# jpreprocess/jbonsai

Measured on AMD Instinct MI355X. Metric: 48 kHz PCM samples/sec (whole node), batched utterances, higher is better.
Workload: dtype f64

## Files before the change

jbonsai_amd/csrc/jb_mlpg.hip:

```cpp
#include "jb_device.h"

#include <cstdlib>
#include <type_traits>

namespace jb {

__device__ __forceinline__ uint32_t ps_scan_incl(uint32_t v, int lane)
{
#pragma unroll
    for (int o = 1; o < 64; o <<= 1) {
        const uint32_t u = (uint32_t)__shfl_up((int)v, o);
        if (lane >= o)
            v += u;
    }
    return v;
}

__global__ __launch_bounds__(64) void k_prep_states(BatchDev bd, StreamDev sd, int si)
{
    if ((int)blockIdx.x >= bd.B)
        return;
    const int b = (int)bd.order[blockIdx.x];
    const int lane = threadIdx.x;
    const UttDev *up = bd.utt + b;
// ... 1064 lines not shown
        if (p >= 0 && p < nch && lane < L) {
            const long l0 = lo(p);
            const double *ib = inb + (p % kFlIn) * NIN * kFlCT * LP;
            double *ob = outb + (p % kFlOut) * NOUT * kFlCT * LP;
            constexpr int kHalf = kFlCT / 2;
            const bool interior = l0 >= 2 && l0 + kFlCT + 2 <= (long)n;
#pragma unroll
            for (int h = 0; h < 2; h++) {
                double ivs[kHalf][NIN];
#pragma unroll
                for (int uu = 0; uu < kHalf; uu++) {
                    const int u = h * kHalf + uu;
                    const int tt = BACKWARD ? kFlCT - 1 - u : u;
#pragma unroll
                    for (int a = 0; a < NIN; a++)
                        ivs[uu][a] = ib[(a * kFlCT + tt) * LP + lane];
                }
                __builtin_amdgcn_sched_barrier(0);
                if (interior) {
#pragma unroll
                    for (int uu = 0; uu < kHalf; uu++) {
                        const int u = h * kHalf + uu;
                        const int tt = BACKWARD ? kFlCT - 1 - u : u;
                        double ov[NOUT];
                        step(std::true_type{}, (uint32_t)(l0 + tt), ivs[uu], ov);
#pragma unroll
                        for (int a = 0; a < NOUT; a++)
                            ob[(a * kFlCT + tt) * LP + lane] = ov[a];
                    }
                } else {
#pragma unroll
                    for (int uu = 0; uu < kHalf; uu++) {
                        const int u = h * kHalf + uu;
                        const int tt = BACKWARD ? kFlCT - 1 - u : u;
                        const long t = l0 + tt;
                        if (t >= 0 && t < (long)n) {
                            double ov[NOUT];
                            step(std::false_type{}, (uint32_t)t, ivs[uu], ov);
#pragma unroll
                            for (int a = 0; a < NOUT; a++)
                                ob[(a * kFlCT + tt) * LP + lane] = ov[a];
                        }
                    }
                }
                __builtin_amdgcn_sched_barrier(0);
            }
        }
    };
    auto phase_end = [&]() {
        asm volatile("s_waitcnt lgkmcnt(0)" ::: "memory");
        __builtin_amdgcn_s_barrier();
        asm volatile("" ::: "memory");
    };
    static_assert(kFlGroups == 3 && kFlOut == 3, "roles: park c-2 / drain c+2 fall on different groups for 3");
    for (int p = -2 - kFlGroups; p <= nch + 1; p++) {
        if (solver)
            solver_phase(p);
        else
            mover_phase(p);
        phase_end();
    }
}

template <int LMAX>
__global__ __launch_bounds__(kFlNT, 1) void k_mlpg_fb_lds(BatchDev bd, StreamDev sd, int si)
{
    extern __shared__ double lds[];
    const int b = (int)bd.order[blockIdx.x];
    const UttDev *up = bd.utt + b;
    const uint32_t n = sd.Tv[b];
    if (n == 0)
        return;
    const int L = sd.L;
    const uint64_t row0 = mt_row0(up, L);
    const uint64_t rs = up->mt_rs;
    if (threadIdx.x < 64)
        __builtin_amdgcn_s_setprio(3);
    else
        __builtin_amdgcn_s_setprio(2);
    {
        const double *const in[4] = {sd.A[0] + row0, sd.A[1] + row0, sd.A[2] + row0, sd.bvec + row0};
        double *const out[3] = {sd.F[1] + row0, sd.F[2] + row0, sd.g + row0};
        double p1_0 = 0, p1_1 = 0, p1_2 = 0, p2_0 = 0, p2_2 = 0, g1 = 0, g2 = 0;
        fl_pass<LMAX, 4, 3, false>(lds, in, out, n, L, rs,
                                   [&](auto interior, uint32_t t, const double (&iv)[4], double (&ov)[3]) {
            constexpr bool IN = decltype(interior)::value;
            double r0 = iv[0], r1 = iv[1], r2 = iv[2], g = iv[3];
            if (IN || t >= 1)
                r0 -= p1_1 * p1_1 * p1_0;
            if (IN || t >= 2)
                r0 -= p2_2 * p2_2 * p2_0;
            if (IN || t >= 1)
                r1 -= p1_1 * p1_2 * p1_0;
            const double rr = fb_rcp(r0);
            r1 = fb_div(r1, r0, rr);
            r2 = fb_div(r2, r0, rr);
            if (IN || t >= 1)
                g -= p1_1 * g1;
            if (IN || t >= 2)
                g -= p2_2 * g2;
            ov[0] = r1;
            ov[1] = r2;
            ov[2] = fb_div(g, r0, rr);
            p2_0 = p1_0;
            p2_2 = p1_2;
            g2 = g1;
            p1_0 = r0;
            p1_1 = r1;
            p1_2 = r2;
            g1 = g;
        });
    }
    __threadfence();
    __syncthreads();
    {
        const double *const in[3] = {sd.F[1] + row0, sd.F[2] + row0, sd.g + row0};
        double *const out[1] = {sd.par + row0};
        double q1 = 0, q2 = 0;
        fl_pass<LMAX, 3, 1, true>(lds, in, out, n, L, rs,
                                  [&](auto interior, uint32_t t, const double (&iv)[3], double (&ov)[1]) {
            constexpr bool IN = decltype(interior)::value;
            double p = iv[2];
            if (IN || t + 1 < n)
                p -= iv[0] * q1;
            if (IN || t + 2 < n)
                p -= iv[1] * q2;
            ov[0] = p;
            q2 = q1;
            q1 = p;
        });
    }
}

constexpr int kFrCh = 8;
constexpr int kFrPitch = kFrCh + 1;
__global__ __launch_bounds__(64) void k_mlpg_fb_runs(BatchDev bd, StreamDev sd, int si)
{
    const int b = (int)bd.order[blockIdx.y];
    const UttDev *up = bd.utt + b;
    const int lane = threadIdx.x;
    const uint32_t r = blockIdx.x * 64u + (uint32_t)lane;
    const uint32_t nr = sd.nruns[b];
    if (blockIdx.x * 64u >= nr)
        return;
    const uint64_t base = up->frame_off, sb = up->state_off;
    const uint32_t T = up->T;
    uint32_t k0 = 0, len = 0;
    if (r < nr) {
        const uint32_t t0 = sd.run_list[sb + r];
        const bool ok = t0 < T && sd.voiced[base + t0] && !(t0 > 0 && sd.voiced[base + t0 - 1]) &&
                        !(r > 0 && sd.run_list[sb + r - 1] == t0);
        if (ok) {
            const uint32_t s0 = sd.fstate[base + t0];
            k0 = sd.s_vpre[sb + s0] + (t0 - sd.s_start[sb + s0]);
            len = sd.s_rend[sb + s0] - t0 + 1;
        }
    }
    __shared__ uint32_t rk0[64], rlen[64];
    __shared__ double img[4][64][kFrPitch];
    rk0[lane] = k0;
    rlen[lane] = len;
    uint32_t maxlen = len;
    for (int o = 32; o > 0; o >>= 1)
        maxlen = max(maxlen, (uint32_t)__shfl_xor((int)maxlen, o));
    if (maxlen == 0)
        return;
    const uint32_t nch = (maxlen + kFrCh - 1) / kFrCh;
    auto wsync = [] {
        __builtin_amdgcn_fence(__ATOMIC_RELEASE, "wavefront");
        __builtin_amdgcn_wave_barrier();
        __builtin_amdgcn_fence(__ATOMIC_ACQUIRE, "wavefront");
    };
    wsync();
    const int sub = lane & 7, grp = lane >> 3;
    const double *const in4[4] = {sd.A[0] + base, sd.A[1] + base, sd.A[2] + base, sd.bvec + base};
    double *const f4[4] = {sd.F[0] + base, sd.F[1] + base, sd.F[2] + base, sd.g + base};
    auto fetch = [&](const double *const (&arr)[4], uint32_t c, double (&v)[4][8]) {
#pragma unroll
        for (int j = 0; j < 8; j++) {
            const int rr = 8 * j + grp;
            const uint32_t t = c * kFrCh + (uint32_t)sub;
            const bool in = t < rlen[rr];
            const uint64_t o = (uint64_t)rk0[rr] + (in ? t : 0u);
#pragma unroll
            for (int a = 0; a < 4; a++)
                v[a][j] = arr[a][o];
        }
    };
    auto park = [&](const double (&v)[4][8]) {
#pragma unroll
        for (int j = 0; j < 8; j++)
#pragma unroll
            for (int a = 0; a < 4; a++)
                img[a][8 * j + grp][sub] = v[a][j];
    };
    auto drain = [&](double *const *arr, int na, uint32_t c) {
#pragma unroll
        for (int j = 0; j < 8; j++) {
            const int rr = 8 * j + grp;
            const uint32_t t = c * kFrCh + (uint32_t)sub;
            if (t < rlen[rr]) {
                const uint64_t o = (uint64_t)rk0[rr] + t;
                for (int a = 0; a < na; a++)
                    arr[a][o] = img[a][rr][sub];
            }
        }
    };
    {
        double p1_0 = 0, p1_1 = 0, p1_2 = 0, p2_0 = 0, p2_2 = 0, g1 = 0, g2 = 0;
        double v[4][8];
        fetch(in4, 0, v);
        for (uint32_t c = 0; c < nch; c++) {
            wsync();
            park(v);
            if (c + 1 < nch)
                fetch(in4, c + 1, v);
            wsync();
            const uint32_t tb = c * kFrCh;
#pragma unroll
            for (int i = 0; i < kFrCh; i++) {
                const uint32_t t = tb + (uint32_t)i;
                if (t < len) {
                    double r0 = img[0][lane][i], r1 = img[1][lane][i], r2 = img[2][lane][i], g = img[3][lane][i];
                    if (t >= 1)
                        r0 -= p1_1 * p1_1 * p1_0;
                    if (t >= 2)
                        r0 -= p2_2 * p2_2 * p2_0;
                    if (t >= 1)
                        r1 -= p1_1 * p1_2 * p1_0;
                    const double rr = fb_rcp(r0);
                    r1 = fb_div(r1, r0, rr);
                    r2 = fb_div(r2, r0, rr);
                    if (t >= 1)
                        g -= p1_1 * g1;
                    if (t >= 2)
                        g -= p2_2 * g2;
                    img[0][lane][i] = r0;
                    img[1][lane][i] = r1;
                    img[2][lane][i] = r2;
                    img[3][lane][i] = g;
                    p2_0 = p1_0;
                    p2_2 = p1_2;
                    g2 = g1;
                    p1_0 = r0;
                    p1_1 = r1;
                    p1_2 = r2;
                    g1 = g;
                }
            }
            wsync();
            drain(f4, 4, c);
        }
    }
    __threadfence_block();
    wsync();
    {
        double q1 = 0, q2 = 0;
        double v[4][8];
        double *const p1[1] = {sd.par + base};
        const double *const fr4[4] = {sd.F[0] + base, sd.F[1] + base, sd.F[2] + base, sd.g + base};
        fetch(fr4, nch - 1, v);
        for (uint32_t c = nch; c-- > 0;) {
            wsync();
            park(v);
            if (c > 0)
                fetch(fr4, c - 1, v);
            wsync();
            const uint32_t tb = c * kFrCh;
#pragma unroll
            for (int i = kFrCh - 1; i >= 0; i--) {
                const uint32_t t = tb + (uint32_t)i;
                if (t < len) {
                    const double d = img[0][lane][i];
                    double p = fb_div(img[3][lane][i], d, fb_rcp(d));
                    if (t + 1 < len)
                        p -= img[1][lane][i] * q1;
                    if (t + 2 < len)
                        p -= img[2][lane][i] * q2;
                    img[0][lane][i] = p;
                    q2 = q1;
                    q1 = p;
                }
            }
            wsync();
            drain(p1, 1, c);
        }
    }
}

__device__ __forceinline__ double rl64(double v, int lane)
{
    int lo = __builtin_amdgcn_readlane(__double2loint(v), lane);
    int hi = __builtin_amdgcn_readlane(__double2hiint(v), lane);
    return __hiloint2double(hi, lo);
}
__device__ __forceinline__ double serial_add64(double acc, double v)
{
#pragma unroll
    for (int u = 0; u < 64; u++)
        acc += rl64(v, u);
    return acc;
}

#ifndef JB_VT_NB
#define JB_VT_NB 8
#endif
constexpr int kVtNB = JB_VT_NB;

__device__ __forceinline__ double serial_add_lds(double acc, const double *buf)
{
    const double2 *b2 = reinterpret_cast<const double2 *>(buf);
    double2 x[2][8];
#pragma unroll
    for (int u = 0; u < 8; u++)
        x[0][u] = b2[u];
#pragma unroll
    for (int g = 0; g < 4; g++) {
        if (g < 3) {
#pragma unroll
            for (int u = 0; u < 8; u++)
                x[(g + 1) & 1][u] = b2[8 * (g + 1) + u];
        }
        __builtin_amdgcn_sched_barrier(0);
#pragma unroll
        for (int u = 0; u < 8; u++) {
            acc += x[g & 1][u].x;
            acc += x[g & 1][u].y;
        }
        __builtin_amdgcn_sched_barrier(0);
    }
    return acc;
}

__device__ __forceinline__ void serial_add2_lds(double &acc_a, const double *buf_a, double &acc_b, const double *buf_b)
{
    const double2 *a2 = reinterpret_cast<const double2 *>(buf_a), *b2 = reinterpret_cast<const double2 *>(buf_b);
    double2 x[2][4], y[2][4];
#pragma unroll
    for (int u = 0; u < 4; u++) {
        x[0][u] = a2[u];
        y[0][u] = b2[u];
    }
#pragma unroll
    for (int g = 0; g < 8; g++) {
        if (g < 7) {
#pragma unroll
            for (int u = 0; u < 4; u++) {
                x[(g + 1) & 1][u] = a2[4 * (g + 1) + u];
                y[(g + 1) & 1][u] = b2[4 * (g + 1) + u];
            }
        }
        __builtin_amdgcn_sched_barrier(0);
#pragma unroll
        for (int u = 0; u < 4; u++) {
            acc_a += x[g & 1][u].x;
            acc_b += y[g & 1][u].x;
            acc_a += x[g & 1][u].y;
            acc_b += y[g & 1][u].y;
        }
        __builtin_amdgcn_sched_barrier(0);
    }
}

template <bool NONMSD>
__global__ __launch_bounds__(64) void k_mlpg_gv_vt(BatchDev bd, StreamDev sd, int si)
{
    const int m = blockIdx.x, b = (int)bd.order[blockIdx.y], lane = threadIdx.x;
    const UttDev *up = bd.utt + b;
    const StreamStatesDev st = up->st[si];
    const uint32_t n = sd.Tv[b];
    const uint32_t gvl = sd.gvlen[b];
    if (n == 0 || !(sd.use_gv && st.gv_mean && gvl > 0))
        return;
    const int L = sd.L;
    const uint64_t base = up->frame_off;
    const uint64_t o0 = base * (uint64_t)L + (uint64_t)m, Ls = (uint64_t)L;
#define IX(k) (o0 + (uint64_t)(k) * Ls)
    __shared__ __attribute__((aligned(16))) double sbuf[2][kVtNB][64];
    const uint8_t *sw = sd.vsw + base;
    const double *A0 = sd.A[0], *A1 = sd.A[1], *A2 = sd.A[2], *Bv = sd.bvec;
    double *Gv = sd.g, *Pv = sd.par, *Ov = sd.out;
    const double gv_mean = st.gv_mean[m] * st.gv_weight;
    const double gv_vari = st.gv_var[m];
    const double glen = (double)gvl;
    constexpr uint32_t STEP = 64u * kVtNB;

    double ssum = 0.0;
    for (uint32_t tb = 0; tb < n; tb += STEP) {
        double v[kVtNB];
#pragma unroll
        for (int q = 0; q < kVtNB; q++) {
            const uint32_t t = tb + 64u * q + (uint32_t)lane;
            v[q] = (t < n && sw[t]) ? Pv[IX(t)] : 0.0;
        }
        __syncthreads();
#pragma unroll
        for (int q = 0; q < kVtNB; q++)
            sbuf[0][q][lane] = v[q];
        __syncthreads();
#pragma unroll
        for (int q = 0; q < kVtNB; q++)
            if (tb + 64u * q < n)
                ssum = serial_add_lds(ssum, sbuf[0][q]);
    }
    double mean = ssum / glen;
    double vsum = 0.0;
    for (uint32_t tb = 0; tb < n; tb += STEP) {
        double v[kVtNB];
#pragma unroll
        for (int q = 0; q < kVtNB; q++) {
            const uint32_t t = tb + 64u * q + (uint32_t)lane;
            const bool on = t < n && sw[t];
            const double p = on ? Pv[IX(t)] : mean;
            v[q] = on ? (p - mean) * (p - mean) : 0.0;
        }
        __syncthreads();
#pragma unroll
        for (int q = 0; q < kVtNB; q++)
            sbuf[0][q][lane] = v[q];
        __syncthreads();
#pragma unroll
        for (int q = 0; q < kVtNB; q++)
            if (tb + 64u * q < n)
                vsum = serial_add_lds(vsum, sbuf[0][q]);
    }
    double vari = vsum / glen;
    {
        const double ratio = sqrt(gv_mean / vari);
        ssum = 0.0;
        for (uint32_t tb = 0; tb < n; tb += STEP) {
            double v[kVtNB];
#pragma unroll
            for (int q = 0; q < kVtNB; q++) {
                const uint32_t t = tb + 64u * q + (uint32_t)lane;
                const bool on = t < n && sw[t];
                double pn = 0.0;
                if (on) {
                    pn = ratio * (Pv[IX(t)] - mean) + mean;
                    Pv[IX(t)] = pn;
                }
                v[q] = pn;
            }
        __syncthreads();
#pragma unroll
        for (int q = 0; q < kVtNB; q++)
            sbuf[0][q][lane] = v[q];
        __syncthreads();
#pragma unroll
        for (int q = 0; q < kVtNB; q++)
            if (tb + 64u * q < n)
                ssum = serial_add_lds(ssum, sbuf[0][q]);
        }
    }
    double step = 0.1, prev = 0.0;
    const double length = (double)n;
    const double wgt = 1.0 / (double)((uint64_t)sd.W * (uint64_t)n);
    const double ll = (double)((uint64_t)n * (uint64_t)n);
    const double lm1 = (double)(n - 1);
    for (int it = 1; it <= 5; it++) {
        mean = ssum / glen;
        double hmmobj = 0.0;
        vsum = 0.0;
        __syncthreads();
        for (uint32_t tb = 0; tb < n; tb += STEP) {
            double vs[kVtNB], hv[kVtNB];
            double l_p0[kVtNB], l_pp1[kVtNB], l_pm1[kVtNB], l_pp2[kVtNB], l_pm2[kVtNB], l_a0[kVtNB],
                l_a1[kVtNB], l_a1m[kVtNB], l_a2[kVtNB], l_a2m[kVtNB], l_b[kVtNB];
            uint8_t l_sw[kVtNB];
#pragma unroll
            for (int q = 0; q < kVtNB; q++) {
                const uint32_t t = tb + 64u * q + (uint32_t)lane;
                const uint32_t tc = t < n ? t : n - 1;
                const uint32_t t1 = tc + 1 < n ? tc + 1 : n - 1, t2 = tc + 2 < n ? tc + 2 : n - 1;
                const uint32_t m1 = tc >= 1 ? tc - 1 : 0, m2 = tc >= 2 ? tc - 2 : 0;
                l_p0[q] = Pv[IX(tc)];
                l_pp1[q] = Pv[IX(t1)];
                l_pm1[q] = Pv[IX(m1)];
                l_pp2[q] = Pv[IX(t2)];
                l_pm2[q] = Pv[IX(m2)];
                l_a0[q] = A0[IX(tc)];
                l_a1[q] = A1[IX(tc)];
                l_a1m[q] = A1[IX(m1)];
                l_a2[q] = A2[IX(tc)];
                l_a2m[q] = A2[IX(m2)];
                l_b[q] = Bv[IX(tc)];
                l_sw[q] = sw[tc];
            }
#pragma unroll
            for (int q = 0; q < kVtNB; q++) {
                const uint32_t t = tb + 64u * q + (uint32_t)lane;
                vs[q] = hv[q] = 0.0;
                if (t < n) {
                    const double p0 = l_p0[q];
                    if (l_sw[q])
                        vs[q] = (p0 - mean) * (p0 - mean);
                    double g = l_a0[q] * p0;
                    if (t + 1 < n)
                        g += l_a1[q] * l_pp1[q];
                    if (t >= 1)
                        g += l_a1m[q] * l_pm1[q];
                    if (t + 2 < n)
                        g += l_a2[q] * l_pp2[q];
                    if (t >= 2)
                        g += l_a2m[q] * l_pm2[q];
                    Gv[IX(t)] = g;
                    hv[q] = 1.0 * wgt * p0 * (l_b[q] - 0.5 * g);
                }
            }
            __syncthreads();
#pragma unroll
            for (int q = 0; q < kVtNB; q++) {
                sbuf[0][q][lane] = vs[q];
                sbuf[1][q][lane] = hv[q];
            }
            __syncthreads();
#pragma unroll
            for (int q = 0; q < kVtNB; q++)
                if (tb + 64u * q < n) {
                    serial_add2_lds(vsum, sbuf[0][q], hmmobj, sbuf[1][q]);
                }
        }
        vari = vsum / glen;
        const double gvobj = -0.5 * 1.0 * vari * gv_vari * (vari - 2.0 * gv_mean);
        const double obj = -(hmmobj + gvobj);
        if (it > 1) {
            if (obj > prev)
                step *= 0.5;
            else if (obj < prev)
                step *= 1.2;
        }
        const double dv = -2.0 * gv_vari * (vari - gv_mean) / length;
        ssum = 0.0;
        __syncthreads();
        for (uint32_t tb = 0; tb < n; tb += STEP) {
            double sn[kVtNB];
            double l_p[kVtNB], l_a0[kVtNB], l_g[kVtNB], l_b[kVtNB];
            uint8_t l_sw[kVtNB];
#pragma unroll
            for (int q = 0; q < kVtNB; q++) {
                const uint32_t t = tb + 64u * q + (uint32_t)lane;
                const uint32_t tc = t < n ? t : n - 1;
                l_p[q] = Pv[IX(tc)];
                l_a0[q] = A0[IX(tc)];
                l_g[q] = Gv[IX(tc)];
                l_b[q] = Bv[IX(tc)];
                l_sw[q] = sw[tc];
            }
#pragma unroll
            for (int q = 0; q < kVtNB; q++) {
                const uint32_t t = tb + 64u * q + (uint32_t)lane;
                sn[q] = 0.0;
                if (t < n) {
                    const double p = l_p[q];
                    const double h = -1.0 * wgt * l_a0[q] -
                                     1.0 * 2.0 / ll *
                                         (lm1 * gv_vari * (vari - gv_mean) +
                                          2.0 * gv_vari * (p - mean) * (p - mean));
                    const bool on = l_sw[q] != 0;
                    double next_g;
                    if (on)
                        next_g = 1.0 / h * (1.0 * wgt * (-l_g[q] + l_b[q]) + 1.0 * dv * (p - mean));
                    else
                        next_g = 1.0 / h * (1.0 * wgt * (-l_g[q] + l_b[q]));
                    const double pnew = p + step * next_g;
                    if (NONMSD && it == 5)
                        Ov[IX(t)] = pnew;
                    else
                        Pv[IX(t)] = pnew;
                    if (on)
                        sn[q] = pnew;
                }
            }
        __syncthreads();
#pragma unroll
        for (int q = 0; q < kVtNB; q++)
            sbuf[0][q][lane] = sn[q];
        __syncthreads();
#pragma unroll
        for (int q = 0; q < kVtNB; q++)
            if (tb + 64u * q < n)
                ssum = serial_add_lds(ssum, sbuf[0][q]);
        }
        prev = obj;
    }
#undef IX
}

constexpr int kGvTT = 2048;
constexpr int kGvNT = 512;
constexpr int kGvKX = (kGvTT + 4 + kGvNT - 1) / kGvNT;

struct GvScal {
    double mean, vari, step, obj;
};

template <int MODE, bool IN>
__device__ __forceinline__ void gv_tp_body(const BatchDev &bd, const StreamDev &sd, int si, int it,
                                           const double *__restrict__ src, double *__restrict__ dst,
                                           int stats, const UttDev *up, uint32_t n, uint32_t gvl, int t0)
{
    const int tile = blockIdx.x, m = blockIdx.y, b = blockIdx.z, tid = threadIdx.x;
    const StreamStatesDev st = up->st[si];
    if (!st.gv_mean)
        return;
    const int L = sd.L, B = bd.B;
    const uint32_t NT = sd.gv_ntile;
    const uint64_t row = mt_row0(up, L) + (uint64_t)m * (uint64_t)up->mt_rs;
    const uint8_t *sw = sd.vsw + up->frame_off;
    const double *A0 = sd.A[0] + row, *A1 = sd.A[1] + row, *A2 = sd.A[2] + row, *Bv = sd.bvec + row;
    const double *P = src + row;
    double *Q = dst ? dst + row : nullptr;

    constexpr int KW = (kGvTT + 8 + kGvNT - 1) / kGvNT;
    double pw[KW], a0r[kGvKX], a1r[kGvKX], a2r[kGvKX], a1m[kGvKX], a2m[kGvKX], br[kGvKX];
    bool onr[kGvKX];
    double p_own[kGvTT / kGvNT];
    bool on_own[kGvTT / kGvNT];
    if (MODE == 0) {
#pragma unroll
        for (int k = 0; k < kGvTT / kGvNT; k++) {
            const uint32_t t = (uint32_t)t0 + (uint32_t)(tid + kGvNT * k);
            const bool ok = IN || t < n;
            p_own[k] = ok ? P[t] : 0.0;
            on_own[k] = ok && sw[t] != 0;
        }
    } else {
#pragma unroll
        for (int k = 0; k < KW; k++) {
            const int i = tid + kGvNT * k;
            const int t = t0 - 4 + i;
            const bool ok = i < kGvTT + 8 && (IN || (t >= 0 && (uint32_t)t < n));
            pw[k] = ok ? P[t] : 0.0;
        }
#pragma unroll
        for (int k = 0; k < kGvKX; k++) {
            const int i = tid + kGvNT * k;
            const int t = t0 - 2 + i;
            const bool ok = i < kGvTT + 4 && (IN || (t >= 0 && (uint32_t)t < n));
            a0r[k] = ok ? A0[t] : 0.0;
            a1r[k] = ok ? A1[t] : 0.0;
            a2r[k] = ok ? A2[t] : 0.0;
            a1m[k] = (ok && (IN || t >= 1)) ? A1[t - 1] : 0.0;
            a2m[k] = (ok && (IN || t >= 2)) ? A2[t - 2] : 0.0;
            br[k] = ok ? Bv[t] : 0.0;
            onr[k] = ok && sw[t] != 0;
        }
    }

    const double gv_mean = st.gv_mean[m] * st.gv_weight;
    const double gv_vari = st.gv_var[m];
    const double glen = (double)gvl;
    const uint32_t ntile_b = (n + kGvTT - 1) / kGvTT;
    const uint64_t bl = (uint64_t)b * L + m;
    auto part = [&](int pass) { return sd.gv_part + (((uint64_t)pass * B * L + bl) * NT) * 4; };
    auto scal = [&](int k) { return sd.gv_scal + ((uint64_t)k * B * L + bl) * 4; };

    double K = 0.0, mean = 0.0, vari = 0.0, ratio = 1.0, step = 0.0;
    if (MODE == 0) {
        K = P[0];
    } else {
        const double *pp = part(MODE == 1 ? 0 : it);
        double S1 = 0.0, S2 = 0.0, H = 0.0;
        for (uint32_t j = 0; j < ntile_b; j++) {
            S1 += pp[4 * j + 0];
            S2 += pp[4 * j + 1];
            H += pp[4 * j + 2];
        }
        const double Kprev = (MODE == 1) ? P[0] : scal(it - 1)[0];
        mean = Kprev + S1 / glen;
        vari = (S2 - S1 * S1 / glen) / glen;
        K = mean;
        if (MODE == 1) {
            ratio = sqrt(gv_mean / vari);
            if (tile == 0 && tid == 0) {
                double *sc = scal(0);
                sc[0] = mean;
                sc[1] = 0.1;
                sc[2] = 0.0;
            }
        } else {
            const double gvobj = -0.5 * 1.0 * vari * gv_vari * (vari - 2.0 * gv_mean);
            const double obj = -(H + gvobj);
            step = 0.1;
            if (it > 1) {
                const double prev = scal(it - 1)[2];
                step = scal(it - 1)[1];
                if (obj > prev)
                    step *= 0.5;
                else if (obj < prev)
                    step *= 1.2;
            }
            if (tile == 0 && tid == 0) {
                double *sc = scal(it);
                sc[0] = mean;
                sc[1] = step;
                sc[2] = obj;
            }
        }
    }
    const double wgt = 1.0 / (double)((uint64_t)sd.W * (uint64_t)n);

    double s1 = 0.0, s2 = 0.0, hh = 0.0;
    if (MODE == 0) {
#pragma unroll
        for (int k = 0; k < kGvTT / kGvNT; k++) {
            if (on_own[k]) {
                const double dlt = p_own[k] - K;
                s1 += dlt;
                s2 += dlt * dlt;
            }
        }
    } else {
        __shared__ double po[kGvTT + 8], pn[kGvTT + 4];
#pragma unroll
        for (int k = 0; k < KW; k++) {
            const int i = tid + kGvNT * k;
            if (i < kGvTT + 8)
                po[i] = pw[k];
        }
        __syncthreads();
        const double length = (double)n;
        const double ll = (double)((uint64_t)n * (uint64_t)n);
        const double lm1 = (double)(n - 1);
        const double dv = -2.0 * gv_vari * (vari - gv_mean) / length;
#pragma unroll
        for (int k = 0; k < kGvKX; k++) {
            const int i = tid + kGvNT * k;
            const int t = t0 - 2 + i;
            if (i < kGvTT + 4 && (IN || (t >= 0 && (uint32_t)t < n))) {
                const double p = po[i + 2];
                const bool on = onr[k];
                const double a0 = a0r[k], bb = br[k];
                double pnew;
                if (MODE == 1) {
                    pnew = on ? ratio * (p - mean) + mean : p;
                } else {
                    double g = a0 * p;
                    if (IN || (uint32_t)t + 1 < n)
                        g += a1r[k] * po[i + 3];
                    if (IN || t >= 1)
                        g += a1m[k] * po[i + 1];
                    if (IN || (uint32_t)t + 2 < n)
                        g += a2r[k] * po[i + 4];
                    if (IN || t >= 2)
                        g += a2m[k] * po[i];
                    const double h = -1.0 * wgt * a0 -
                                     1.0 * 2.0 / ll *
                                         (lm1 * gv_vari * (vari - gv_mean) +
                                          2.0 * gv_vari * (p - mean) * (p - mean));
                    double next_g;
                    if (on)
                        next_g = 1.0 / h * (1.0 * wgt * (-g + bb) + 1.0 * dv * (p - mean));
                    else
                        next_g = 1.0 / h * (1.0 * wgt * (-g + bb));
                    pnew = p + step * next_g;
                }
                pn[i] = pnew;
            }
        }
        __syncthreads();
#pragma unroll
        for (int k = 0; k < kGvKX; k++) {
            const int i = tid + kGvNT * k;
            const int t = t0 - 2 + i;
            if (i >= 2 && i < kGvTT + 2 && (IN || (uint32_t)t < n)) {
                const double p0 = pn[i];
                Q[t] = p0;
                if (stats) {
                    if (onr[k]) {
                        const double dlt = p0 - K;
                        s1 += dlt;
                        s2 += dlt * dlt;
                    }
                    double g = a0r[k] * p0;
                    if (IN || (uint32_t)t + 1 < n)
                        g += a1r[k] * pn[i + 1];
                    if (IN || t >= 1)
                        g += a1m[k] * pn[i - 1];
                    if (IN || (uint32_t)t + 2 < n)
                        g += a2r[k] * pn[i + 2];
                    if (IN || t >= 2)
                        g += a2m[k] * pn[i - 2];
                    hh += 1.0 * wgt * p0 * (br[k] - 0.5 * g);
                }
            }
        }
    }
    if (!stats)
        return;
#pragma unroll
    for (int o = 32; o > 0; o >>= 1) {
        s1 += __shfl_xor(s1, o);
        s2 += __shfl_xor(s2, o);
        hh += __shfl_xor(hh, o);
    }
    __shared__ double red[kGvNT / 64][3];
    if ((tid & 63) == 0) {
        red[tid >> 6][0] = s1;
        red[tid >> 6][1] = s2;
        red[tid >> 6][2] = hh;
    }
    __syncthreads();
    if (tid == 0) {
        double r0 = red[0][0], r1 = red[0][1], r2 = red[0][2];
#pragma unroll
        for (int w = 1; w < kGvNT / 64; w++) {
            r0 += red[w][0];
            r1 += red[w][1];
            r2 += red[w][2];
        }
        double *po_ = part(MODE == 0 ? 0 : (MODE == 1 ? 1 : it + 1)) + 4 * (uint64_t)tile;
        po_[0] = r0;
        po_[1] = r1;
        po_[2] = r2;
    }
}

template <int MODE>
__global__ __launch_bounds__(kGvNT) void k_mlpg_gv_tp(BatchDev bd, StreamDev sd, int si, int it,
                                                       const double *__restrict__ src,
                                                       double *__restrict__ dst, int stats)
{
    const int b = blockIdx.z;
    const UttDev *up = bd.utt + b;
    const uint32_t n = sd.Tv[b], gvl = sd.gvlen[b];
    const int t0 = blockIdx.x * kGvTT;
    if (n == 0 || gvl == 0 || (uint32_t)t0 >= n)
        return;
    if (t0 >= 4 && (uint32_t)t0 + kGvTT + 4 <= n)
        gv_tp_body<MODE, true>(bd, sd, si, it, src, dst, stats, up, n, gvl, t0);
    else
        gv_tp_body<MODE, false>(bd, sd, si, it, src, dst, stats, up, n, gvl, t0);
}

__global__ __launch_bounds__(256) void k_mlpg_scatter_mt(BatchDev bd, StreamDev sd)
{
    extern __shared__ double tile[];
    const int b = blockIdx.y;
    const UttDev *up = bd.utt + b;
    const uint32_t T = up->T;
    const uint32_t t0 = blockIdx.x * 64u;
    if (t0 >= T)
        return;
    const uint64_t base = up->frame_off, sb = up->state_off;
    const int L = sd.L;
    for (int e = threadIdx.x; e < 64 * L; e += blockDim.x) {
        const int m = e >> 6, tl = e & 63;
        const uint32_t t = t0 + (uint32_t)tl;
        double v = kNoData;
        if (t < T && sd.voiced[base + t]) {
            uint32_t k = t;
            if (sd.is_msd) {
                const uint32_t s_ = sd.fstate[base + t];
                k = sd.s_vpre[sb + s_] + (t - sd.s_start[sb + s_]);
            }
            v = sd.par[mt_row0(up, L) + (uint64_t)m * up->mt_rs + k];
        }
        tile[m * 65 + tl] = v;
    }
    __syncthreads();
    const uint32_t nt = T - t0 < 64u ? T - t0 : 64u;
    for (int e = threadIdx.x; e < (int)nt * L; e += blockDim.x) {
        const int tl = e / L, m = e % L;
        sd.out[(base + t0 + (uint32_t)tl) * (uint64_t)L + (uint64_t)m] = tile[m * 65 + tl];
    }
}

__global__ void k_mlpg_scatter(BatchDev bd, StreamDev sd)
{
    const int b = blockIdx.y;
    const UttDev *up = bd.utt + b;
    const uint32_t T = up->T;
    const uint64_t base = up->frame_off, sb = up->state_off;
    const int L = sd.L;
    const uint64_t tid = (uint64_t)blockIdx.x * blockDim.x + threadIdx.x;
    if (tid >= (uint64_t)T * L)
        return;
    const uint32_t t = (uint32_t)(tid / L);
    const int m = (int)(tid % L);
    double v = kNoData;
    if (sd.voiced[base + t]) {
        const uint32_t s_ = sd.fstate[base + t];
        const uint32_t k = sd.s_vpre[sb + s_] + (t - sd.s_start[sb + s_]);
        v = sd.par[(base + k) * (uint64_t)L + (uint64_t)m];
    }
    sd.out[(base + t) * (uint64_t)L + (uint64_t)m] = v;
}

hipError_t launch_prep(const BatchDev &bd, const StreamDev &sd, int si, hipStream_t stream)
{
    if (bd.B == 0)
        return hipSuccess;
    {
        dim3 grid(bd.B), block(64);
        if (!sd.is_msd)
            hipLaunchKernelGGL(k_prep_states_dense, grid, block, 0, stream, bd, sd, si);
        else
            hipLaunchKernelGGL(k_prep_states, grid, block, 0, stream, bd, sd, si);
    }
    if (bd.maxS > 0) {
        dim3 grid((bd.maxS + 127) / 128, bd.B), block(128);
        hipLaunchKernelGGL(k_prep_frames, grid, block, 0, stream, bd, sd, si);
    }
    return hipGetLastError();
}

template <int LMAX>
static void launch_fb_lds(const BatchDev &bd, const StreamDev &sd, int si, size_t lds, hipStream_t stream)
{
    static const hipError_t attr = hipFuncSetAttribute((const void *)k_mlpg_fb_lds<LMAX>,
                                                       hipFuncAttributeMaxDynamicSharedMemorySize, 160 * 1024);
    (void)attr;
    hipLaunchKernelGGL(k_mlpg_fb_lds<LMAX>, dim3(bd.B), dim3(kFlNT), lds, stream, bd, sd, si);
}

static void launch_fb(const BatchDev &bd, const StreamDev &sd, int si, hipStream_t stream)
{
    constexpr size_t lds1 = sizeof(double) * (size_t)(kFlIn * 4 + kFlOut * 3) * kFlCT;
    static_assert(lds1 * kMtMaxDim <= 160 * 1024, "the widest [dim][frame] stream must fit the LDS of a CU");
    if (sd.L == 1)
        launch_fb_lds<1>(bd, sd, si, lds1, stream);
    else if (sd.L <= 36)
        launch_fb_lds<36>(bd, sd, si, lds1 * 37, stream);
    else
        launch_fb_lds<64>(bd, sd, si, lds1 * (size_t)sd.L, stream);
}

template <int BW>
static hipError_t launch_mlpg_bw(const BatchDev &bd, const StreamDev &sd, int si, hipStream_t stream,
                                 hipEvent_t after_build, jb_enqueue_hook &between, void *between_ctx,
                                 hipEvent_t after_ivar)
{
    const uint64_t work = (uint64_t)bd.maxT * (uint64_t)sd.L;
    if (work == 0 || bd.B == 0)
        return hipSuccess;
    if constexpr (BW == 3) if (sd.mt) {
        {
            const uint64_t ne = (uint64_t)bd.maxS * (uint64_t)(sd.W * sd.L);
            constexpr uint64_t per = 256u * kIvarPer;
            dim3 grid((unsigned)((ne + per - 1) / per), bd.B), block(256);
            hipLaunchKernelGGL(k_mlpg_ivar, grid, block, 0, stream, bd, sd, si);
            if (after_ivar)
                (void)hipEventRecord(after_ivar, stream);
        }
        {
            dim3 grid((bd.maxT + kBuildTF - 1) / kBuildTF, bd.B);
            const size_t lds = sizeof(double) * (size_t)(BW + 1) * sd.L * (kBuildTF + 1);
            const int nthr = ((kBuildTF / kBuildRun) * sd.L + 63) / 64 * 64;
            JB_DBG_SKIP_IF(si == 0 ? 1 : 0, hipLaunchKernelGGL(k_mlpg_build_mt2<BW>, grid, dim3((unsigned)nthr), lds, stream, bd, sd, si));
        }
        if (after_build)
            (void)hipEventRecord(after_build, stream);
        dim3 grid((sd.L + 63) / 64, bd.B), block(64);
        const bool tp = sd.use_gv && !sd.serial_gv && sd.gv_part;
        if (sd.is_msd) {
            if (tp)
                launch_fb(bd, sd, si, stream);
            else
                hipLaunchKernelGGL((k_mlpg_solve3<false, true, true>), grid, block, 0, stream, bd, sd, si);
        } else {
            if (tp)
                JB_DBG_SKIP_IF(si == 0 ? 2 : 0, launch_fb(bd, sd, si, stream));
            else
                hipLaunchKernelGGL((k_mlpg_solve3<true, true, true>), grid, block, 0, stream, bd, sd, si);
        }
        if (between) {
            hipError_t he = between(between_ctx, stream);
            if (he != hipSuccess)
                return he;
            between = nullptr;
        }
        if (tp && sd.gv_gang_ctl) {
            hipError_t he = hipSuccess;
            JB_DBG_SKIP_IF(16, he = launch_gv_gang(bd, sd, si, stream));
            if (he != hipSuccess)
                return he;
        } else if (tp && sd.gv_gsweep) {
            hipError_t he = launch_gv_gsweep(bd, sd, si, stream);
            if (he != hipSuccess)
                return he;
        } else if (tp) {
            dim3 gg(sd.gv_ntile, sd.L, bd.B), gb(kGvNT);
            hipLaunchKernelGGL(k_mlpg_gv_tp<0>, gg, gb, 0, stream, bd, sd, si, 0, sd.par, (double *)nullptr, 1);
            hipLaunchKernelGGL(k_mlpg_gv_tp<1>, gg, gb, 0, stream, bd, sd, si, 0, sd.par, sd.g, 1);
            for (int it = 1; it <= 5; it++) {
                const double *src = (it & 1) ? sd.g : sd.par;
                double *dst = (it & 1) ? sd.par : sd.g;
                hipLaunchKernelGGL(k_mlpg_gv_tp<2>, gg, gb, 0, stream, bd, sd, si, it, src, dst, it < 5 ? 1 : 0);
            }
        }
        if (!sd.defer_out) {
            dim3 g2((bd.maxT + 63) / 64, bd.B), b2(256);
            hipLaunchKernelGGL(k_mlpg_scatter_mt, g2, b2, sizeof(double) * (size_t)sd.L * 65, stream, bd, sd);
        }
        return hipGetLastError();
    }
    {
        dim3 grid((unsigned)((work + 255) / 256), bd.B), block(256);
        hipLaunchKernelGGL(k_mlpg_build<BW>, grid, block, 0, stream, bd, sd, si);
    }
    if (after_build)
        (void)hipEventRecord(after_build, stream);
    {
        dim3 grid((sd.L + 63) / 64, bd.B), block(64);
        if (BW == 3 && !sd.generic_solver) {
            const bool gv_vt = sd.use_gv && sd.L <= 2;
            dim3 gvgrid(sd.L, bd.B);
            if (sd.is_msd) {
                if (gv_vt) {
                    if (sd.L == 1 && sd.win_width[0] == 1) {
                        dim3 rg((bd.maxS + 63) / 64, bd.B);
                        JB_DBG_SKIP_IF(128, hipLaunchKernelGGL(k_mlpg_fb_runs, rg, dim3(64), 0, stream, bd, sd, si));
                    } else
                        hipLaunchKernelGGL((k_mlpg_solve3<false, false>), grid, block, 0, stream, bd, sd, si);
                    JB_DBG_SKIP_IF(32, hipLaunchKernelGGL(k_mlpg_gv_vt<false>, gvgrid, block, 0, stream, bd, sd, si));
                } else {
                    hipLaunchKernelGGL((k_mlpg_solve3<false, true>), grid, block, 0, stream, bd, sd, si);
                }
                dim3 g2((unsigned)((work + 255) / 256), bd.B), b2(256);
                hipLaunchKernelGGL(k_mlpg_scatter, g2, b2, 0, stream, bd, sd);
            } else if (gv_vt) {
                hipLaunchKernelGGL((k_mlpg_solve3<true, false>), grid, block, 0, stream, bd, sd, si);
                hipLaunchKernelGGL(k_mlpg_gv_vt<true>, gvgrid, block, 0, stream, bd, sd, si);
            } else {
                hipLaunchKernelGGL((k_mlpg_solve3<true, true>), grid, block, 0, stream, bd, sd, si);
            }
        } else {
            hipLaunchKernelGGL(k_mlpg_solve<BW>, grid, block, 0, stream, bd, sd, si);
        }
    }
    return hipGetLastError();
}

__global__ __launch_bounds__(256) void k_mc2b_mt(BatchDev bd, StreamDev sd, VocDev vd, int write_out)
{
    extern __shared__ double tile[];
    const int b = blockIdx.y;
    const UttDev *up = bd.utt + b;
    const uint32_t T = up->T;
    const uint32_t t0 = blockIdx.x * 64u;
    if (t0 >= T)
        return;
    const uint64_t base = up->frame_off;
    const int L = sd.L;
    const uint32_t nt = T - t0 < 64u ? T - t0 : 64u;
    for (int e = threadIdx.x; e < 64 * L; e += blockDim.x) {
        const int m = e >> 6, tl = e & 63;
        tile[m * 65 + tl] = (uint32_t)tl < nt ? sd.par[mt_row0(up, L) + (uint64_t)m * up->mt_rs + t0 + (uint32_t)tl] : 0.0;
    }
    __syncthreads();
    const uint64_t o0 = (base + t0) * (uint64_t)L;
    if (write_out)
        for (int e = threadIdx.x; e < (int)nt * L; e += blockDim.x)
            sd.out[o0 + (uint64_t)e] = tile[(e % L) * 65 + e / L];
    __syncthreads();
    const double alpha = voc_alpha(vd, (uint32_t)b);
    if (threadIdx.x < nt && alpha != 0.0) {
        const int tl = threadIdx.x;
        double prev = tile[(L - 1) * 65 + tl];
        for (int i = L - 2; i >= 0; i--) {
            prev = tile[i * 65 + tl] - alpha * prev;
            tile[i * 65 + tl] = prev;
        }
    }
    __syncthreads();
    for (int e = threadIdx.x; e < (int)nt * L; e += blockDim.x)
        vd.bcoef[o0 + (uint64_t)e] = tile[(e % L) * 65 + e / L];
}

hipError_t launch_mc2b_mt(const BatchDev &bd, const StreamDev &sd, const VocDev &vd, bool write_out,
                          hipStream_t stream)
{
    if (bd.B == 0 || bd.maxT == 0)
        return hipSuccess;
    dim3 grid((bd.maxT + 63) / 64, bd.B), block(256);
    hipLaunchKernelGGL(k_mc2b_mt, grid, block, sizeof(double) * (size_t)sd.L * 65, stream, bd, sd, vd,
                       write_out ? 1 : 0);
    return hipGetLastError();
}

constexpr double kHalfToneMinLf0 = 2.995732273553991;
constexpr double kHalfToneMaxLf0 = 9.903487552536127;
__global__ __launch_bounds__(256) void k_gather_blend(const GatherJob *__restrict__ jobs)
{
    const GatherJob &j = jobs[blockIdx.y];
    const uint64_t e = (uint64_t)blockIdx.x * blockDim.x + threadIdx.x;
    if (e >= (uint64_t)j.S * j.WL)
        return;
    const uint32_t s = (uint32_t)(e / j.WL), k = (uint32_t)(e % j.WL);
    const float *p0 = j.tab[0] + (uint64_t)j.row[0][s] * j.row_len;
    double m = (double)p0[k] * j.w[0], v = (double)p0[j.WL + k] * j.w[0];
    double q = (j.has_msd && k == 0) ? (double)p0[2 * j.WL] * j.w[0] : 0.0;
    for (uint32_t vi = 1; vi < j.nv; vi++) {
        const float *p = j.tab[vi] + (uint64_t)j.row[vi][s] * j.row_len;
        m += j.w[vi] * (double)p[k];
        v += j.w[vi] * (double)p[j.WL + k];
        if (j.has_msd && k == 0)
            q += j.w[vi] * (double)p[2 * j.WL];
    }
    if (j.lf0_offset != 0.0 && k == 0) {
        const double x = m + j.lf0_offset;
        m = fmin(fmax(x, kHalfToneMinLf0), kHalfToneMaxLf0);
    }
    j.mean[e] = m;
    j.var[e] = v;
    if (j.has_msd && k == 0 && j.msd)
        j.msd[s] = q;
}

hipError_t launch_gather(const GatherJob *jobs_dev, uint32_t n_jobs, uint64_t max_elems, hipStream_t stream)
{
    if (n_jobs == 0 || max_elems == 0)
        return hipSuccess;
    dim3 grid((unsigned)((max_elems + 255) / 256), n_jobs), block(256);
    hipLaunchKernelGGL(k_gather_blend, grid, block, 0, stream, jobs_dev);
    return hipGetLastError();
}

int mlpg_mt_max_dim() { return kMtMaxDim; }
int mlpg_gv_tile_frames() { return kGvTT; }

static hipError_t launch_mlpg_inner(const BatchDev &bd, const StreamDev &sd, int si, hipStream_t stream,
                                    hipEvent_t after_build, jb_enqueue_hook &between, void *between_ctx,
                                    hipEvent_t after_ivar);

hipError_t launch_mlpg(const BatchDev &bd, const StreamDev &sd, int si, hipStream_t stream, hipEvent_t after_build,
                       jb_enqueue_hook between, void *between_ctx, hipEvent_t after_ivar)
{
    hipError_t e = launch_mlpg_inner(bd, sd, si, stream, after_build, between, between_ctx, after_ivar);
    if (e == hipSuccess && between)
        e = between(between_ctx, stream);
    return e;
}

static hipError_t launch_mlpg_inner(const BatchDev &bd, const StreamDev &sd, int si, hipStream_t stream,
                                    hipEvent_t after_build, jb_enqueue_hook &between, void *between_ctx,
                                    hipEvent_t after_ivar)
{
    if (after_ivar && !(sd.BW == 3 && sd.mt))
        (void)hipEventRecord(after_ivar, stream);
    if (sd.is_static()) {
        const uint64_t work = (uint64_t)bd.maxT * (uint64_t)sd.L;
        if (work == 0 || bd.B == 0)
            return hipSuccess;
        dim3 grid((unsigned)((work + 255) / 256), bd.B), block(256);
        if (sd.canon && sd.canon_n && sd.L <= 32) {
            dim3 grid_rows((bd.maxT + 7) / 8, bd.B);
            JB_DBG_SKIP_IF(256, hipLaunchKernelGGL(k_mlpg_static_rows, grid_rows, block, 0, stream, bd, sd, si));
            if (after_build)
                (void)hipEventRecord(after_build, stream);
            return hipGetLastError();
        }
        if (sd.canon && sd.canon_n) {
            hipError_t e = hipMemsetAsync(sd.canon, 1, sd.canon_n, stream);
            if (e != hipSuccess)
                return e;
        }
        JB_DBG_SKIP_IF(256, hipLaunchKernelGGL(k_mlpg_static, grid, block, 0, stream, bd, sd, si));
        if (after_build)
            (void)hipEventRecord(after_build, stream);
        return hipGetLastError();
    }
    switch (sd.BW) {
    case 1:
        return launch_mlpg_bw<1>(bd, sd, si, stream, after_build, between, between_ctx, after_ivar);
    case 3:
        return launch_mlpg_bw<3>(bd, sd, si, stream, after_build, between, between_ctx, after_ivar);
    case 5:
        return launch_mlpg_bw<5>(bd, sd, si, stream, after_build, between, between_ctx, after_ivar);
    case 7:
        return launch_mlpg_bw<7>(bd, sd, si, stream, after_build, between, between_ctx, after_ivar);
    case 9:
        return launch_mlpg_bw<9>(bd, sd, si, stream, after_build, between, between_ctx, after_ivar);
    default:
        return hipErrorInvalidValue;
    }
}

}
```

Baseline: 20.50 billion.

## Split GV kernel into producer waves and a serial-adder wave with LDS ring

Measured after the change: 20.66 billion, median of 6. About the same (+0.8%).

```diff
diff --git a/jbonsai_amd/csrc/jb_mlpg.hip b/jbonsai_amd/csrc/jb_mlpg.hip
--- a/jbonsai_amd/csrc/jb_mlpg.hip
+++ b/jbonsai_amd/csrc/jb_mlpg.hip
@@ -1390,10 +1390,9 @@
     return acc;
 }
 
-#ifndef JB_VT_NB
-#define JB_VT_NB 8
-#endif
-constexpr int kVtNB = JB_VT_NB;
+constexpr int kVtNB = 4;
+constexpr int kVtProd = 3;
+constexpr int kVtNT = 64 * (1 + kVtProd);
 
 __device__ __forceinline__ double serial_add_lds(double acc, const double *buf)
 {
@@ -1451,9 +1450,11 @@
 }
 
 template <bool NONMSD>
-__global__ __launch_bounds__(64) void k_mlpg_gv_vt(BatchDev bd, StreamDev sd, int si)
-{
-    const int m = blockIdx.x, b = (int)bd.order[blockIdx.y], lane = threadIdx.x;
+__global__ __launch_bounds__(kVtNT) __attribute__((amdgpu_waves_per_eu(3, 3))) void k_mlpg_gv_vt(BatchDev bd, StreamDev sd, int si)
+{
+    const int m = blockIdx.x, b = (int)bd.order[blockIdx.y];
+    int lane = threadIdx.x & 63;
+    const int wv = __builtin_amdgcn_readfirstlane((int)(threadIdx.x >> 6));
     const UttDev *up = bd.utt + b;
     const StreamStatesDev st = up->st[si];
     const uint32_t n = sd.Tv[b];
@@ -1464,7 +1465,8 @@
     const uint64_t base = up->frame_off;
     const uint64_t o0 = base * (uint64_t)L + (uint64_t)m, Ls = (uint64_t)L;
 #define IX(k) (o0 + (uint64_t)(k) * Ls)
-    __shared__ __attribute__((aligned(16))) double sbuf[2][kVtNB][64];
+    __shared__ __attribute__((aligned(16))) double ring[2][kVtProd][2 * kVtNB * 64];
+    __shared__ double sc[4];
     const uint8_t *sw = sd.vsw + base;
     const double *A0 = sd.A[0], *A1 = sd.A[1], *A2 = sd.A[2], *Bv = sd.bvec;
     double *Gv = sd.g, *Pv = sd.par, *Ov = sd.out;
@@ -1472,73 +1474,115 @@
     const double gv_vari = st.gv_var[m];
     const double glen = (double)gvl;
     constexpr uint32_t STEP = 64u * kVtNB;
-
-    double ssum = 0.0;
-    for (uint32_t tb = 0; tb < n; tb += STEP) {
-        double v[kVtNB];
+    const uint32_t nch = (n + STEP - 1) / STEP;
+    const bool adder = wv == 0;
+    if (adder)
+        __builtin_amdgcn_s_setprio(3);
+    else
+        __builtin_amdgcn_s_setprio(2);
+
+    const uint32_t nrd = (nch + (uint32_t)kVtProd - 1) / (uint32_t)kVtProd;
+    auto phase_end = [&]() {
+        asm volatile("s_waitcnt lgkmcnt(0)" ::: "memory");
+        __builtin_amdgcn_s_barrier();
+        asm volatile("" ::: "memory");
+    };
+    auto sweep = [&](auto load, auto produce, auto add) {
+        if (adder) {
+            for (uint32_t r = 0; r <= nrd; r++) {
+                if (r >= 1) {
+#pragma unroll
+                    for (int k = 0; k < kVtProd; k++)
+                        add((r - 1) * (uint32_t)kVtProd + (uint32_t)k, ring[(r - 1) & 1][k]);
+                }
+                phase_end();
+            }
+        } else {
+            uint32_t c = (uint32_t)(wv - 1);
+            load(c < nch ? c : nch - 1);
+            for (uint32_t r = 0; r <= nrd; r++) {
+                if (c < nch)
+                    produce(c, ring[r & 1][wv - 1]);
+                __builtin_amdgcn_sched_barrier(0);
+                c += (uint32_t)kVtProd;
+                load(c < nch ? c : nch - 1);
+                phase_end();
+            }
+        }
+    };
+    double acc = 0.0, acc2 = 0.0;
+    auto add1 = [&](uint32_t c, const double *slot) {
+#pragma unroll
+        for (int q = 0; q < kVtNB; q++)
+            if (c * STEP + 64u * q < n)
+                acc = serial_add_lds(acc, slot + 64 * q);
+    };
+    auto add2 = [&](uint32_t c, const double *slot) {
+#pragma unroll
+        for (int q = 0; q < kVtNB; q++)
+            if (c * STEP + 64u * q < n)
+                serial_add2_lds(acc, slot + 64 * q, acc2, slot + 64 * (kVtNB + q));
+    };
+    double l_p[kVtNB];
+    uint8_t l_sw[kVtNB];
+    auto load_p = [&](uint32_t c) {
 #pragma unroll
         for (int q = 0; q < kVtNB; q++) {
-            const uint32_t t = tb + 64u * q + (uint32_t)lane;
-            v[q] = (t < n && sw[t]) ? Pv[IX(t)] : 0.0;
-        }
-        __syncthreads();
-#pragma unroll
-        for (int q = 0; q < kVtNB; q++)
-            sbuf[0][q][lane] = v[q];
-        __syncthreads();
-#pragma unroll
-        for (int q = 0; q < kVtNB; q++)
-            if (tb + 64u * q < n)
-                ssum = serial_add_lds(ssum, sbuf[0][q]);
-    }
-    double mean = ssum / glen;
-    double vsum = 0.0;
-    for (uint32_t tb = 0; tb < n; tb += STEP) {
-        double v[kVtNB];
-#pragma unroll
-        for (int q = 0; q < kVtNB; q++) {
-            const uint32_t t = tb + 64u * q + (uint32_t)lane;
-            const bool on = t < n && sw[t];
-            const double p = on ? Pv[IX(t)] : mean;
-            v[q] = on ? (p - mean) * (p - mean) : 0.0;
-        }
-        __syncthreads();
-#pragma unroll
-        for (int q = 0; q < kVtNB; q++)
-            sbuf[0][q][lane] = v[q];
-        __syncthreads();
-#pragma unroll
-        for (int q = 0; q < kVtNB; q++)
-            if (tb + 64u * q < n)
-                vsum = serial_add_lds(vsum, sbuf[0][q]);
-    }
-    double vari = vsum / glen;
+            const uint32_t t = c * STEP + 64u * q + (uint32_t)lane;
+            const uint32_t tc = t < n ? t : n - 1;
+            l_p[q] = Pv[IX(tc)];
+            l_sw[q] = sw[tc];
+        }
+    };
+
+    sweep(load_p,
+          [&](uint32_t c, double *slot) {
+#pragma unroll
+              for (int q = 0; q < kVtNB; q++) {
+                  const uint32_t t = c * STEP + 64u * q + (uint32_t)lane;
+                  slot[64 * q + lane] = (t < n && l_sw[q]) ? l_p[q] : 0.0;
+              }
+          },
+          add1);
+    if (adder)
+        sc[0] = acc / glen;
+    __syncthreads();
+    double mean = sc[0];
+    acc = 0.0;
+    sweep(load_p,
+          [&](uint32_t c, double *slot) {
+#pragma unroll
+              for (int q = 0; q < kVtNB; q++) {
+                  const uint32_t t = c * STEP + 64u * q + (uint32_t)lane;
+                  const bool on = t < n && l_sw[q];
+                  const double p = on ? l_p[q] : mean;
+                  slot[64 * q + lane] = on ? (p - mean) * (p - mean) : 0.0;
+              }
+          },
+          add1);
+    if (adder) {
+        const double vari = acc / glen;
+        sc[1] = sqrt(gv_mean / vari);
+    }
+    __syncthreads();
     {
-        const double ratio = sqrt(gv_mean / vari);
-        ssum = 0.0;
-        for (uint32_t tb = 0; tb < n; tb += STEP) {
-            double v[kVtNB];
-#pragma unroll
-            for (int q = 0; q < kVtNB; q++) {
-                const uint32_t t = tb + 64u * q + (uint32_t)lane;
-                const bool on = t < n && sw[t];
-                double pn = 0.0;
-                if (on) {
-                    pn = ratio * (Pv[IX(t)] - mean) + mean;
-                    Pv[IX(t)] = pn;
-                }
-                v[q] = pn;
-            }
-        __syncthreads();
-#pragma unroll
-        for (int q = 0; q < kVtNB; q++)
-            sbuf[0][q][lane] = v[q];
-        __syncthreads();
-#pragma unroll
-        for (int q = 0; q < kVtNB; q++)
-            if (tb + 64u * q < n)
-                ssum = serial_add_lds(ssum, sbuf[0][q]);
-        }
+        const double ratio = sc[1];
+        acc = 0.0;
+        sweep(load_p,
+              [&](uint32_t c, double *slot) {
+#pragma unroll
+                  for (int q = 0; q < kVtNB; q++) {
+                      const uint32_t t = c * STEP + 64u * q + (uint32_t)lane;
+                      const bool on = t < n && l_sw[q];
+                      double pn = 0.0;
+                      if (on) {
+                          pn = ratio * (l_p[q] - mean) + mean;
+                          Pv[IX(t)] = pn;
+                      }
+                      slot[64 * q + lane] = pn;
+                  }
+              },
+              add1);
     }
     double step = 0.1, prev = 0.0;
     const double length = (double)n;
@@ -1546,128 +1590,127 @@
     const double ll = (double)((uint64_t)n * (uint64_t)n);
     const double lm1 = (double)(n - 1);
     for (int it = 1; it <= 5; it++) {
-        mean = ssum / glen;
-        double hmmobj = 0.0;
-        vsum = 0.0;
+        asm volatile("" : "+v"(lane));
+        if (adder)
+            sc[0] = acc / glen;
         __syncthreads();
-        for (uint32_t tb = 0; tb < n; tb += STEP) {
-            double vs[kVtNB], hv[kVtNB];
-            double l_p0[kVtNB], l_pp1[kVtNB], l_pm1[kVtNB], l_pp2[kVtNB], l_pm2[kVtNB], l_a0[kVtNB],
-                l_a1[kVtNB], l_a1m[kVtNB], l_a2[kVtNB], l_a2m[kVtNB], l_b[kVtNB];
-            uint8_t l_sw[kVtNB];
-#pragma unroll
-            for (int q = 0; q < kVtNB; q++) {
-                const uint32_t t = tb + 64u * q + (uint32_t)lane;
-                const uint32_t tc = t < n ? t : n - 1;
-                const uint32_t t1 = tc + 1 < n ? tc + 1 : n - 1, t2 = tc + 2 < n ? tc + 2 : n - 1;
-                const uint32_t m1 = tc >= 1 ? tc - 1 : 0, m2 = tc >= 2 ? tc - 2 : 0;
-                l_p0[q] = Pv[IX(tc)];
-                l_pp1[q] = Pv[IX(t1)];
-                l_pm1[q] = Pv[IX(m1)];
-                l_pp2[q] = Pv[IX(t2)];
-                l_pm2[q] = Pv[IX(m2)];
-                l_a0[q] = A0[IX(tc)];
-                l_a1[q] = A1[IX(tc)];
-                l_a1m[q] = A1[IX(m1)];
-                l_a2[q] = A2[IX(tc)];
-                l_a2m[q] = A2[IX(m2)];
-                l_b[q] = Bv[IX(tc)];
-                l_sw[q] = sw[tc];
-            }
-#pragma unroll
-            for (int q = 0; q < kVtNB; q++) {
-                const uint32_t t = tb + 64u * q + (uint32_t)lane;
-                vs[q] = hv[q] = 0.0;
-                if (t < n) {
-                    const double p0 = l_p0[q];
-                    if (l_sw[q])
-                        vs[q] = (p0 - mean) * (p0 - mean);
-                    double g = l_a0[q] * p0;
-                    if (t + 1 < n)
-                        g += l_a1[q] * l_pp1[q];
-                    if (t >= 1)
-                        g += l_a1m[q] * l_pm1[q];
-                    if (t + 2 < n)
-                        g += l_a2[q] * l_pp2[q];
-                    if (t >= 2)
-                        g += l_a2m[q] * l_pm2[q];
-                    Gv[IX(t)] = g;
-                    hv[q] = 1.0 * wgt * p0 * (l_b[q] - 0.5 * g);
-                }
-            }
-            __syncthreads();
-#pragma unroll
-            for (int q = 0; q < kVtNB; q++) {
-                sbuf[0][q][lane] = vs[q];
-                sbuf[1][q][lane] = hv[q];
-            }
-            __syncthreads();
-#pragma unroll
-            for (int q = 0; q < kVtNB; q++)
-                if (tb + 64u * q < n) {
-                    serial_add2_lds(vsum, sbuf[0][q], hmmobj, sbuf[1][q]);
-                }
-        }
-        vari = vsum / glen;
-        const double gvobj = -0.5 * 1.0 * vari * gv_vari * (vari - 2.0 * gv_mean);
-        const double obj = -(hmmobj + gvobj);
-        if (it > 1) {
-            if (obj > prev)
-                step *= 0.5;
-            else if (obj < prev)
-                step *= 1.2;
-        }
-        const double dv = -2.0 * gv_vari * (vari - gv_mean) / length;
-        ssum = 0.0;
+        mean = sc[0];
+        acc = 0.0;
+        acc2 = 0.0;
+        {
+            double l_pp1[kVtNB], l_pm1[kVtNB], l_pp2[kVtNB], l_pm2[kVtNB], l_a0[kVtNB], l_a1[kVtNB],
+                l_a1m[kVtNB], l_a2[kVtNB], l_a2m[kVtNB], l_b[kVtNB];
+            sweep(
+                [&](uint32_t c) {
+#pragma unroll
+                    for (int q = 0; q < kVtNB; q++) {
+                        const uint32_t t = c * STEP + 64u * q + (uint32_t)lane;
+                        const uint32_t tc = t < n ? t : n - 1;
+                        const uint32_t t1 = tc + 1 < n ? tc + 1 : n - 1, t2 = tc + 2 < n ? tc + 2 : n - 1;
+                        const uint32_t m1 = tc >= 1 ? tc - 1 : 0, m2 = tc >= 2 ? tc - 2 : 0;
+                        l_p[q] = Pv[IX(tc)];
+                        l_pp1[q] = Pv[IX(t1)];
+                        l_pm1[q] = Pv[IX(m1)];
+                        l_pp2[q] = Pv[IX(t2)];
+                        l_pm2[q] = Pv[IX(m2)];
+                        l_a0[q] = A0[IX(tc)];
+                        l_a1[q] = A1[IX(tc)];
+                        l_a1m[q] = A1[IX(m1)];
+                        l_a2[q] = A2[IX(tc)];
+                        l_a2m[q] = A2[IX(m2)];
+                        l_b[q] = Bv[IX(tc)];
+                        l_sw[q] = sw[tc];
+                    }
+                },
+                [&](uint32_t c, double *slot) {
+#pragma unroll
+                    for (int q = 0; q < kVtNB; q++) {
+                        const uint32_t t = c * STEP + 64u * q + (uint32_t)lane;
+                        double vs = 0.0, hv = 0.0;
+                        if (t < n) {
+                            const double p0 = l_p[q];
+                            if (l_sw[q])
+                                vs = (p0 - mean) * (p0 - mean);
+                            double g = l_a0[q] * p0;
+                            if (t + 1 < n)
+                                g += l_a1[q] * l_pp1[q];
+                            if (t >= 1)
+                                g += l_a1m[q] * l_pm1[q];
+                            if (t + 2 < n)
+                                g += l_a2[q] * l_pp2[q];
+                            if (t >= 2)
+                                g += l_a2m[q] * l_pm2[q];
+                            Gv[IX(t)] = g;
+                            hv = 1.0 * wgt * p0 * (l_b[q] - 0.5 * g);
+                        }
+                        slot[64 * q + lane] = vs;
+                        slot[64 * (kVtNB + q) + lane] = hv;
+                    }
+                },
+                add2);
+        }
+        double obj = 0.0;
+        if (adder) {
+            const double vari = acc / glen;
+            const double gvobj = -0.5 * 1.0 * vari * gv_vari * (vari - 2.0 * gv_mean);
+            obj = -(acc2 + gvobj);
+            if (it > 1) {
+                if (obj > prev)
+                    step *= 0.5;
+                else if (obj < prev)
+                    step *= 1.2;
+            }
+            sc[1] = vari;
+            sc[2] = step;
+            sc[3] = -2.0 * gv_vari * (vari - gv_mean) / length;
+        }
         __syncthreads();
-        for (uint32_t tb = 0; tb < n; tb += STEP) {
-            double sn[kVtNB];
-            double l_p[kVtNB], l_a0[kVtNB], l_g[kVtNB], l_b[kVtNB];
-            uint8_t l_sw[kVtNB];
-#pragma unroll
-            for (int q = 0; q < kVtNB; q++) {
-                const uint32_t t = tb + 64u * q + (uint32_t)lane;
-                const uint32_t tc = t < n ? t : n - 1;
-                l_p[q] = Pv[IX(tc)];
-                l_a0[q] = A0[IX(tc)];
-                l_g[q] = Gv[IX(tc)];
-                l_b[q] = Bv[IX(tc)];
-                l_sw[q] = sw[tc];
-            }
-#pragma unroll
-            for (int q = 0; q < kVtNB; q++) {
-                const uint32_t t = tb + 64u * q + (uint32_t)lane;
-                sn[q] = 0.0;
-                if (t < n) {
-                    const double p = l_p[q];
-                    const double h = -1.0 * wgt * l_a0[q] -
-                                     1.0 * 2.0 / ll *
-                                         (lm1 * gv_vari * (vari - gv_mean) +
-                                          2.0 * gv_vari * (p - mean) * (p - mean));
-                    const bool on = l_sw[q] != 0;
-                    double next_g;
-                    if (on)
-                        next_g = 1.0 / h * (1.0 * wgt * (-l_g[q] + l_b[q]) + 1.0 * dv * (p - mean));
-                    else
-                        next_g = 1.0 / h * (1.0 * wgt * (-l_g[q] + l_b[q]));
-                    const double pnew = p + step * next_g;
-                    if (NONMSD && it == 5)
-                        Ov[IX(t)] = pnew;
-                    else
-                        Pv[IX(t)] = pnew;
-                    if (on)
-                        sn[q] = pnew;
-                }
-            }
-        __syncthreads();
-#pragma unroll
-        for (int q = 0; q < kVtNB; q++)
-            sbuf[0][q][lane] = sn[q];
-        __syncthreads();
-#pragma unroll
-        for (int q = 0; q < kVtNB; q++)
-            if (tb + 64u * q < n)
-                ssum = serial_add_lds(ssum, sbuf[0][q]);
+        {
+            const double vari = sc[1], stp = sc[2], dv = sc[3];
+            double l_a0[kVtNB], l_g[kVtNB], l_b[kVtNB];
+            acc = 0.0;
+            sweep(
+                [&](uint32_t c) {
+#pragma unroll
+                    for (int q = 0; q < kVtNB; q++) {
+                        const uint32_t t = c * STEP + 64u * q + (uint32_t)lane;
+                        const uint32_t tc = t < n ? t : n - 1;
+                        l_p[q] = Pv[IX(tc)];
+                        l_a0[q] = A0[IX(tc)];
+                        l_g[q] = Gv[IX(tc)];
+                        l_b[q] = Bv[IX(tc)];
+                        l_sw[q] = sw[tc];
+                    }
+                },
+                [&](uint32_t c, double *slot) {
+#pragma unroll
+                    for (int q = 0; q < kVtNB; q++) {
+                        const uint32_t t = c * STEP + 64u * q + (uint32_t)lane;
+                        double sn = 0.0;
+                        if (t < n) {
+                            const double p = l_p[q];
+                            const double h = -1.0 * wgt * l_a0[q] -
+                                             1.0 * 2.0 / ll *
+                                                 (lm1 * gv_vari * (vari - gv_mean) +
+                                                  2.0 * gv_vari * (p - mean) * (p - mean));
+                            const bool on = l_sw[q] != 0;
+                            double next_g;
+                            if (on)
+                                next_g = 1.0 / h * (1.0 * wgt * (-l_g[q] + l_b[q]) + 1.0 * dv * (p - mean));
+                            else
+                                next_g = 1.0 / h * (1.0 * wgt * (-l_g[q] + l_b[q]));
+                            const double pnew = p + stp * next_g;
+                            if (NONMSD && it == 5)
+                                Ov[IX(t)] = pnew;
+                            else
+                                Pv[IX(t)] = pnew;
+                            if (on)
+                                sn = pnew;
+                        }
+                        slot[64 * q + lane] = sn;
+                    }
+                },
+                add1);
         }
         prev = obj;
     }
@@ -2101,7 +2144,7 @@
                         JB_DBG_SKIP_IF(128, hipLaunchKernelGGL(k_mlpg_fb_runs, rg, dim3(64), 0, stream, bd, sd, si));
                     } else
                         hipLaunchKernelGGL((k_mlpg_solve3<false, false>), grid, block, 0, stream, bd, sd, si);
-                    JB_DBG_SKIP_IF(32, hipLaunchKernelGGL(k_mlpg_gv_vt<false>, gvgrid, block, 0, stream, bd, sd, si));
+                    JB_DBG_SKIP_IF(32, hipLaunchKernelGGL(k_mlpg_gv_vt<false>, gvgrid, dim3(kVtNT), 0, stream, bd, sd, si));
                 } else {
                     hipLaunchKernelGGL((k_mlpg_solve3<false, true>), grid, block, 0, stream, bd, sd, si);
                 }
@@ -2109,7 +2152,7 @@
                 hipLaunchKernelGGL(k_mlpg_scatter, g2, b2, 0, stream, bd, sd);
             } else if (gv_vt) {
                 hipLaunchKernelGGL((k_mlpg_solve3<true, false>), grid, block, 0, stream, bd, sd, si);
-                hipLaunchKernelGGL(k_mlpg_gv_vt<true>, gvgrid, block, 0, stream, bd, sd, si);
+                hipLaunchKernelGGL(k_mlpg_gv_vt<true>, gvgrid, dim3(kVtNT), 0, stream, bd, sd, si);
             } else {
                 hipLaunchKernelGGL((k_mlpg_solve3<true, true>), grid, block, 0, stream, bd, sd, si);
             }
```
